# fizzy74/passport-zk-circuits

Hardware: AMD Instinct MI355X
Metric: registerIdentityBuilder witnesses/sec, batch=4096, 1 & 8 MI355X; % HBM roofline (higher is better)
Workload: dtype bn254_fr (u32 limbs)

## Files before the change

passport-zk-circuits_amd/csrc/kernels_rsa.hip:

```cpp
#include <hip/hip_runtime.h>
#include <stdio.h>
#include <stdlib.h>

#define PZK_TEMPLATE_KERNELS_ONLY
#include "regemit.hpp"
#include "rsa_coop.hpp"
#include "kernels.hpp"

namespace pzk {

#define HIP_TRY(x) do { hipError_t e_ = (x); if (e_ != hipSuccess) return e_; } while (0)

template <int K, int G>
static hipError_t launch_rsa_core2(const DevLayout& L, const uint8_t* inputs, uint64_t* rsa_core, int32_t* status,
                                   uint32_t batch, hipStream_t st) {
  constexpr int WPB = 64 / G;
  const size_t lds = sizeof(uint64_t) * rsa2_lds_words<K>() * WPB;
  HIP_TRY(hipFuncSetAttribute((const void*)k_rsa_core2<K, G>, hipFuncAttributeMaxDynamicSharedMemorySize, (int)lds));
  hipLaunchKernelGGL((k_rsa_core2<K, G>), dim3((batch + WPB - 1) / WPB), dim3(64), lds, st, L, inputs, rsa_core, status,
                     batch);
  return hipGetLastError();
}

template <int K, int NL>
static hipError_t launch_rsa_lane(const DevLayout& L, const uint8_t* inputs, uint64_t* rsa_core, uint64_t* colsum,
                                  int32_t* status, uint32_t batch, hipStream_t st) {
  const size_t lds = sizeof(uint64_t) * rsa_lds_words<K>() * NL;
  HIP_TRY(hipFuncSetAttribute((const void*)k_rsa_core<K, NL>, hipFuncAttributeMaxDynamicSharedMemorySize, (int)lds));
  hipLaunchKernelGGL((k_rsa_core<K, NL>), dim3((batch + NL - 1) / NL), dim3(NL), lds, st, L, inputs, rsa_core, colsum,
                     status, batch);
  return hipGetLastError();
}

static bool rsa_core_lane() {
  static const int v = [] {
    const char* e = getenv("PZK_RSA_CORE");
    return e && e[0] == 'l' ? 1 : 0;
  }();
  return v;
}

hipError_t launch_rsa_core(const DevLayout& L, const uint8_t* inputs, uint64_t* rsa_core, uint64_t* colsum,
                           int32_t* status, uint32_t batch, hipStream_t st) {
  const bool lane = rsa_core_lane() && colsum;
  if (L.reg.K == 48) {
    HIP_TRY((launch_rsa_core2<48, 16>(L, inputs, rsa_core, status, batch, st)));
    hipLaunchKernelGGL(k_rsa_inv<48>, dim3((batch + RI_WAVES - 1) / RI_WAVES), dim3(64 * RI_WAVES), 0, st, L, inputs,
                       rsa_core, batch);
  } else if (L.reg.K == 32) {
    HIP_TRY((lane ? launch_rsa_lane<32, 64>(L, inputs, rsa_core, colsum, status, batch, st)
                  : launch_rsa_core2<32, 8>(L, inputs, rsa_core, status, batch, st)));
    hipLaunchKernelGGL(k_rsa_inv<32>, dim3((batch + RI_WAVES - 1) / RI_WAVES), dim3(64 * RI_WAVES), 0, st, L, inputs,
                       rsa_core, batch);
  } else {
    HIP_TRY((lane ? launch_rsa_lane<64, 32>(L, inputs, rsa_core, colsum, status, batch, st)
                  : launch_rsa_core2<64, 16>(L, inputs, rsa_core, status, batch, st)));
    hipLaunchKernelGGL(k_rsa_inv<64>, dim3((batch + RI_WAVES - 1) / RI_WAVES), dim3(64 * RI_WAVES), 0, st, L, inputs,
                       rsa_core, batch);
  }
  return hipGetLastError();
}

hipError_t launch_emit_mm(const DevLayout& L, const Work* work, uint32_t n_work, const Bufs& B, uint32_t batch,
                          hipStream_t st) {
#ifdef PZK_MM_PROF
  {
    static int n = 0;
    if (++n > 1) {
      unsigned long long h[MM_SECTIONS + 2];
      if (hipDeviceSynchronize() == hipSuccess && hipMemcpyFromSymbol(h, HIP_SYMBOL(g_mm_prof), sizeof h) == hipSuccess) {
        fprintf(stderr, "mm_prof launches=%d", n - 1);
        for (int i = 0; i <= (int)MM_SECTIONS; i++) fprintf(stderr, " %llu", h[i]);
        fprintf(stderr, "\n");
      }
    }
  }
#endif
  if (n_work == 0) return hipSuccess;
  const bool m = L.keep.bits != nullptr;
  static const bool wide = !getenv("PZK_MM_THREADS") || atoi(getenv("PZK_MM_THREADS")) != 256;
  const bool w512 = wide && !m && L.reg.K == 32;
  dim3 g(n_work, batch), blk(w512 ? 512 : EMIT_THREADS);
  auto kern = w512 ? k_emit_mm<32, MAP_O0, 512>
            : L.reg.K == 32 ? (m ? k_emit_mm<32, MAP_DIRECT> : k_emit_mm<32, MAP_O0>)
            : L.reg.K == 48 ? (m ? k_emit_mm<48, MAP_DIRECT> : k_emit_mm<48, MAP_O0>)
                            : (m ? k_emit_mm<64, MAP_DIRECT> : k_emit_mm<64, MAP_O0>);
  hipLaunchKernelGGL(kern, g, blk, 0, st, L, work, B);
  return hipGetLastError();
}

}
```

passport-zk-circuits_amd/csrc/regcore.hpp:

```cpp
#pragma once
#include "fr.hpp"
#include "layout.hpp"
#include "poseidon.hpp"
#include "sha.hpp"
#include "core_util.hpp"
#include "pss.hpp"

namespace pzk {

__device__ __forceinline__ fr wave_bits_fr(const uint8_t* row, int base, int L, int dir, bool& bad) {
  const int lane = threadIdx.x & 63;
  fr v = fr_zero();
  for (int q = 0; 64 * q < L; q++) {
    const int k = 64 * q + lane;
    uint32_t b = 0;
    if (k < L) b = in_bit(row, dir > 0 ? base + k : base + L - 1 - k, bad);
    const uint64_t m = __ballot(b);
    v.v[2 * q] = (uint32_t)m;
    v.v[2 * q + 1] = (uint32_t)(m >> 32);
  }
  return v;
}

#ifndef PZK_TEMPLATE_KERNELS_ONLY
// ... 106 lines not shown
    n[i] = in_u64(e);
  }
  int nb = K;
  while (nb > 1 && n[nb - 1] == 0) nb--;
  const int s = __builtin_clzll(n[nb - 1] | 1ull);
  for (int i = nb - 1; i > 0; i--) vn[i] = (n[i] << s) | (s ? n[i - 1] >> (64 - s) : 0ull);
  vn[0] = n[0] << s;
  const uint64_t vtop = vn[nb - 1], vsec = nb > 1 ? vn[nb - 2] : 0ull;
  uint64_t vinv_r;
  const uint64_t vinv = vtop ? divlu(~vtop, ~0ull, vtop, &vinv_r) : 0ull;
  constexpr int MMW = MM_CORE_WORDS(K);
  const int NM = L.reg.n_modmul;
  for (int k = 0; k < NM; k++) {
    uint64_t* mc = core + (size_t)k * MMW;
    for (int i = 0; i < K; i++) {
      uint64_t xi;
      const int sx = L.reg.mm_x[k], sy = L.reg.mm_y[k];
      if (sx < 0) {
        const uint8_t* e = row + 32ull * (L.reg.in_sig + i);
        bad |= !in_is_u64(e);
        xi = in_u64(e);
      } else {
        xi = core[(size_t)sx * MMW + 3 * K + 1 + i];
      }
      uint64_t yi = sy == sx ? xi : core[(size_t)sy * MMW + 3 * K + 1 + i];
      x[i] = xi; y[i] = yi;
      mc[i] = xi; mc[K + i] = yi;
    }
    {
      uint64_t c0 = 0, c1 = 0;
      for (int i = 0; i < 2 * K; i++) {
        U192 acc;
        int lo = i < K ? 0 : i - K + 1, hi = i < K ? i : K - 1;
        for (int j = lo; j <= hi; j++) acc.mac(x[j], y[i - j]);
        if (i < 2 * K - 1) { CS(i, 0) = acc.a0; CS(i, 1) = acc.a1; CS(i, 2) = acc.a2; }
        uint64_t t0 = acc.a0 + c0; uint64_t cc = t0 < c0;
        uint64_t t1 = acc.a1 + c1; uint64_t cc1 = t1 < c1; uint64_t t1b = t1 + cc; cc1 += t1b < t1;
        u[i] = t0; c0 = t1b; c1 = acc.a2 + cc1;
      }
    }
    u[2 * K] = s ? u[2 * K - 1] >> (64 - s) : 0ull;
    if (s) {
      for (int i = 2 * K - 1; i > 0; i--) u[i] = (u[i] << s) | (u[i - 1] >> (64 - s));
      u[0] = u[0] << s;
    }
    for (int j = 0; j <= K; j++) q[j] = 0;
    for (int j = 2 * K - nb; j >= 0 && vtop; j--) {
      uint64_t ujn = u[j + nb], ujn1 = u[j + nb - 1];
      uint64_t qhat, rhat;
      bool rhat_ovf = false;
      if (ujn >= vtop) {
        qhat = ~0ull;
        rhat = ujn1 + vtop;
        rhat_ovf = rhat < ujn1;
      } else {
        qhat = div_preinv(ujn, ujn1, vtop, vinv, &rhat);
      }
      if (nb > 1) {
        for (int it = 0; it < 2 && !rhat_ovf; it++) {
          uint64_t plo = qhat * vsec, phi = __umul64hi(qhat, vsec);
          uint64_t u2 = u[j + nb - 2];
          if (phi > rhat || (phi == rhat && plo > u2)) {
            qhat--;
            uint64_t r2 = rhat + vtop;
            rhat_ovf = r2 < rhat;
            rhat = r2;
          } else {
            break;
          }
        }
      }
      uint64_t borrow = 0, carry = 0;
      for (int i = 0; i < nb; i++) {
        uint64_t plo = qhat * vn[i], phi = __umul64hi(qhat, vn[i]);
        plo += carry; phi += plo < carry; carry = phi;
        uint64_t t = u[i + j];
        uint64_t d = t - plo; uint64_t b1 = t < plo;
        uint64_t d2 = d - borrow; uint64_t b2 = d < borrow;
        u[i + j] = d2; borrow = b1 + b2;
      }
      uint64_t t = u[j + nb];
      uint64_t d = t - carry; uint64_t b1 = t < carry;
      uint64_t d2 = d - borrow; uint64_t b2 = d < borrow;
      u[j + nb] = d2;
      if (b1 + b2) {
        qhat--;
        uint64_t cy = 0;
        for (int i = 0; i < nb; i++) {
          uint64_t a = u[i + j], vb = vn[i];
          uint64_t sm = a + vb; uint64_t ca = sm < a; uint64_t sm2 = sm + cy; uint64_t cb = sm2 < sm;
          u[i + j] = sm2; cy = ca + cb;
        }
        u[j + nb] += cy;
      }
      q[j] = qhat;
    }
    uint64_t* qo = mc + 2 * K;
    uint64_t* ro = mc + 3 * K + 1;
    for (int i = 0; i <= K; i++) qo[i] = q[i];
    for (int i = 0; i < K; i++) {
      uint64_t r = 0;
      if (i < nb) r = s ? (u[i] >> s) | (u[i + 1] << (64 - s)) : u[i];
      ro[i] = r;
    }
    uint64_t* cr = mc + 8 * K + 1;
    {
      uint64_t clo = 0, chi = 0;
      for (int i = 0; i < 2 * K - 1; i++) {
        U192 a, b;
        a.a0 = CS(i, 0); a.a1 = CS(i, 1); a.a2 = CS(i, 2);
        int lo2 = i < K ? 0 : i - K + 1, hi2 = i < K + 1 ? i : K;
        for (int j = lo2; j <= hi2 && j <= K; j++) if (i - j < K) b.mac(q[j], n[i - j]);
        uint64_t s0, s1, s2, s3, br;
        s0 = a.a0 - b.a0; br = a.a0 < b.a0;
        uint64_t t1 = a.a1 - b.a1; uint64_t br1 = a.a1 < b.a1; s1 = t1 - br; br1 += t1 < br; br = br1;
        uint64_t t2 = a.a2 - b.a2; uint64_t br2 = a.a2 < b.a2; s2 = t2 - br; br2 += t2 < br; br = br2;
        s3 = 0 - br;
        uint64_t rr = i < K ? ro[i] : 0ull;
        uint64_t u0 = s0 - rr; uint64_t bb = s0 < rr; s0 = u0;
        uint64_t u1 = s1 - bb; bb = s1 < bb; s1 = u1;
        uint64_t u2 = s2 - bb; bb = s2 < bb; s2 = u2; s3 -= bb;
        uint64_t csx = (int64_t)chi < 0 ? ~0ull : 0ull;
        uint64_t v0 = s0 + clo; uint64_t cc = v0 < s0;
        uint64_t v1 = s1 + chi; uint64_t cc1 = v1 < s1; uint64_t v1b = v1 + cc; cc1 += v1b < v1;
        uint64_t v2 = s2 + csx; uint64_t cc2 = v2 < s2; uint64_t v2b = v2 + cc1; cc2 += v2b < v2;
        uint64_t v3 = s3 + csx + cc2;
        if (i < 2 * K - 2) {
          badz |= v0 != 0;
          clo = v1b; chi = v2b;
          badz |= !((v3 == 0 && (int64_t)v2b >= 0) || (v3 == ~0ull && (int64_t)v2b < 0));
          cr[2 * i] = clo; cr[2 * i + 1] = chi;
        } else {
          badz |= (v0 | v1b | v2b | v3) != 0;
        }
      }
    }
  }
  if (bad || !vtop) set_status(status, ST_INPUT_RANGE);
  if (badz) set_status(status, ST_BIGISZERO);
}

template <int K, int NL>
__global__ void __launch_bounds__(NL) k_rsa_core(DevLayout L, const uint8_t* inputs, uint64_t* rsa_core, uint64_t* colsum,
                                                 int32_t* status, uint32_t batch) {
  core_priority();
  extern __shared__ uint64_t lds_rsa[];
  uint32_t w = blockIdx.x * NL + threadIdx.x;
  if (w >= batch) return;
  rsa_lane<K, NL>(L, inputs + 32ull * (uint64_t)w * L.n_inputs, rsa_core + (size_t)w * L.rsa_core_words, colsum + w,
                  batch, status ? status + w : nullptr, lds_rsa, threadIdx.x);
}

#ifndef PZK_RI_WAVES
#define PZK_RI_WAVES 8
#endif
constexpr int RI_WAVES = PZK_RI_WAVES;
template <int J, int N, class F>
__device__ __forceinline__ void static_for(F&& f) {
  if constexpr (J < N) {
    f(std::integral_constant<int, J>{});
    static_for<J + 1, N>(f);
  }
}
template <int K>
__global__ void __launch_bounds__(64 * RI_WAVES) k_rsa_inv(DevLayout L, const uint8_t* inputs, uint64_t* rsa_core,
                                                           uint32_t batch) {
  core_priority();
  constexpr int PER_MAX = (20 * K + 63) / 64 < 12 ? (20 * K + 63) / 64 : 12;
  __shared__ fr s_tot[RI_WAVES];
  __shared__ fr s_out[RI_WAVES][64];
  const int wv = (int)(threadIdx.x >> 6), lane = (int)(threadIdx.x & 63);
  const uint32_t w0 = blockIdx.x * RI_WAVES + (uint32_t)wv;
  const bool live = w0 < batch;
  const uint32_t w = live ? w0 : batch - 1;
  const int NE = L.reg.n_modmul * K, PER = (NE + 63) / 64, in_pk = (int)L.reg.in_pk;
  constexpr int MMW = MM_CORE_WORDS(K);
  const uint8_t* row = inputs + 32ull * (uint64_t)w * L.n_inputs;
  uint64_t* core = rsa_core + (size_t)w * L.rsa_core_words;
  const int e0 = lane * PER, e1 = !live ? e0 : e0 + PER < NE ? e0 + PER : NE;
  auto diff = [=](int e) -> fr {
    const int k = e / K, i = e - k * K;
    const uint64_t a = core[(size_t)k * MMW + 3 * K + 1 + i], b = in_u64(row + 32ull * (in_pk + i));
    fr d = a >= b ? fr_u64(a - b) : fr_sub(fr_zero(), fr_u64(b - a));
    return fr_to_mont(d);
  };
  auto slot = [=](int e) -> uint8_t* {
    const int k = e / K, i = e - k * K;
    return reinterpret_cast<uint8_t*>(core + (size_t)k * MMW + 4 * K + 1 + 4 * i);
  };
  const bool in_reg = PER <= PER_MAX;
  fr pr[PER_MAX];
  fr acc = fr_mont_one();
  if (in_reg) {
    static_for<0, PER_MAX>([&](auto J) __attribute__((always_inline)) {
      const int e = e0 + J();
      if (e < e1) {
        const fr d = diff(e);
        pr[J()] = acc;
        if (!fr_is_zero(d)) acc = fr_mul_fast(acc, d);
      }
    });
  } else {
    for (int e = e0; e < e1; e++) {
      const fr d = diff(e);
      store_fr(slot(e), acc);
      if (!fr_is_zero(d)) acc = fr_mul_fast(acc, d);
    }
  }
  fr incl = acc, sincl = acc;
  for (int d = 1; d < 64; d <<= 1) {
    fr a = fr_shfl_up(incl, d), b = fr_shfl_down(sincl, d);
    if (lane >= d) incl = fr_mul_fast(incl, a);
    if (lane + d < 64) sincl = fr_mul_fast(sincl, b);
  }
  fr pre = fr_shfl_up(incl, 1), suf = fr_shfl_down(sincl, 1);
  if (lane == 0) pre = fr_mont_one();
  if (lane == 63) suf = fr_mont_one();
  if (lane == 63) s_tot[wv] = incl;
  __syncthreads();
  if (wv == 0) {
    const fr t = lane < RI_WAVES ? s_tot[lane] : fr_mont_one();
    fr t_others, t_all;
    fr_group_others<RI_WAVES>(t, t_others, t_all);
    const fr t_inv = fr_mul_fast(fr_inv<true>(t_all), t_others);
    if (lane < RI_WAVES) s_tot[lane] = t_inv;
  }
  __syncthreads();
  fr inv = fr_mul_fast(fr_mul_fast(s_tot[wv], pre), suf);
  if (!in_reg) {
    if (!live) return;
    for (int e = e1 - 1; e >= e0; e--) {
      const fr d = diff(e);
      fr r = fr_zero();
      if (!fr_is_zero(d)) { r = fr_mul_fast(inv, load_fr(slot(e))); inv = fr_mul_fast(inv, d); }
      store_fr(slot(e), fr_from_mont(r));
    }
    return;
  }
  static_for<0, PER_MAX>([&](auto J) __attribute__((always_inline)) {
    constexpr int j = PER_MAX - 1 - J();
    const int e = e0 + j;
    if (e < e1) {
      const fr d = diff(e);
      fr r = fr_zero();
      if (!fr_is_zero(d)) { r = fr_mul_fast(inv, pr[j]); inv = fr_mul_fast(inv, d); }
      pr[j] = fr_from_mont(r);
    }
  });
  for (int t = 0; t < (NE + 63) / 64; t++) {
    static_for<0, PER_MAX>([&](auto J) __attribute__((always_inline)) {
      const int e = e0 + J();
      if (e < e1 && (e >> 6) == t) s_out[wv][e & 63] = pr[J()];
    });
    __syncthreads();
    const int e = 64 * t + lane;
    if (live && e < NE) store_fr(slot(e), s_out[wv][lane]);
    __syncthreads();
  }
}

constexpr uint64_t RSA_EM4 = 217300885422736416ull, RSA_EM5 = 938447882527703397ull;
constexpr uint64_t RSA_EM6 = 0xFFFFFFFF00303130ull;

#ifndef PZK_TEMPLATE_KERNELS_ONLY
__global__ void __launch_bounds__(64) k_rsa_check(DevLayout L, const uint8_t* inputs, const uint32_t* sha_core,
                                                  const uint64_t* rsa_core, int32_t* status, uint32_t batch) {
  const uint32_t w = blockIdx.x * blockDim.x + threadIdx.x;
  if (w >= batch || !status) return;
  const int K = L.reg.K;
  const uint8_t* row = inputs + 32ull * (uint64_t)w * L.n_inputs;
  const uint64_t* core = rsa_core + (size_t)w * L.rsa_core_words;
  const uint64_t* em = core + (size_t)(L.reg.n_modmul - 1) * MM_CORE_WORDS(K) + 3 * K + 1;
  const ShaJob& J = L.sha[L.reg.j_sa];
  const uint32_t* H = sha_core + (size_t)w * L.sha_core_words + J.hout;
  bool hash_bad = false;
  for (int i = 0; i < 4; i++) {
    const int wd = 3 - i;
    hash_bad |= (((uint64_t)H[2 * wd] << 32) | H[2 * wd + 1]) != em[i];
  }
  bool pad_bad = em[6] != RSA_EM6;
  for (int i = 7; i < K - 1; i++) pad_bad |= em[i] != ~0ull;
  bool gt_bad = false;
  for (int m = 0; m < L.reg.n_modmul; m++) {
    const uint64_t* r = core + (size_t)m * MM_CORE_WORDS(K) + 3 * K + 1;
    int cmp = 0;
    for (int i = K - 1; i >= 0 && cmp == 0; i--) {
      uint64_t n = in_u64(row + 32ull * (L.reg.in_pk + i));
      cmp = n > r[i] ? 1 : n < r[i] ? -1 : 0;
    }
    gt_bad |= cmp != 1;
  }
  if (L.reg.pss_s8) {
    pss_check(pss_view(L, rsa_core, sha_core, w), status + w);
  } else if (J.algo == 1) {
    const uint64_t em2 = em[2];
    if ((uint32_t)em2 != H[0]) lane_status(status + w, ST_RSA_HASH);
    if ((em2 >> 32) != 83887124ull || em[3] != 650212878678426138ull || em[4] != 18446744069417738544ull)
      lane_status(status + w, ST_RSA_PREFIX);
    bool pb = em[K - 1] != 562949953421311ull;
    for (int i = 5; i < K - 1; i++) pb |= em[i] != ~0ull;
    if (pb) lane_status(status + w, ST_RSA_PAD);
  } else {
    if (hash_bad) lane_status(status + w, ST_RSA_HASH);
    if (em[4] != RSA_EM4 || em[5] != RSA_EM5) lane_status(status + w, ST_RSA_PREFIX);
    if (pad_bad) lane_status(status + w, ST_RSA_PAD);
  }
  if (gt_bad) lane_status(status + w, ST_BIGMOD_GT);
}
#endif

struct ExtPt { fr X, Y, Z, T; };

template <class PM = FrMulInline>
__device__ __forceinline__ ExtPt bjj_dbl(const ExtPt& P, const fr& A) {
  fr a = PM::sqr(P.X), b = PM::sqr(P.Y), c = PM::sqr(P.Z);
  c = fr_add(c, c);
  fr d = PM::mul(A, a);
  fr xy = fr_add(P.X, P.Y);
  fr e = fr_sub(fr_sub(PM::sqr(xy), a), b);
  fr g = fr_add(d, b), f = fr_sub(g, c), h = fr_sub(d, b);
  return ExtPt{PM::mul(e, f), PM::mul(g, h), PM::mul(f, g), PM::mul(e, h)};
}
template <class PM = FrMulInline>
__device__ __forceinline__ ExtPt bjj_add_affine(const ExtPt& P, const fr& x2, const fr& y2, const fr& t2d, const fr& A) {
  fr a = PM::mul(P.X, x2), b = PM::mul(P.Y, y2), c = PM::mul(P.T, t2d), d = P.Z;
  fr e = fr_sub(fr_sub(PM::mul(fr_add(P.X, P.Y), fr_add(x2, y2)), a), b);
  fr f = fr_sub(d, c), g = fr_add(d, c), h = fr_sub(b, PM::mul(A, a));
  return ExtPt{PM::mul(e, f), PM::mul(g, h), PM::mul(f, g), PM::mul(e, h)};
}

constexpr uint32_t BJJ_B8X[8] = {0xbb957051u, 0x2893f3f6u, 0x0534e0b6u, 0x2ab8d801u,
                                 0x9d6277c1u, 0x4eacb2e0u, 0xd63e739bu, 0x0bb77a6au};
constexpr uint32_t BJJ_B8Y[8] = {0x872d7d8bu, 0x4b3c257au, 0xb9e13377u, 0xfce0051fu,
                                 0xd16bf9edu, 0x25572e1cu, 0xf7a0b249u, 0x25797203u};
constexpr uint32_t BJJ_INV_B8X[8] = {0x7bc45854u, 0x42cd5135u, 0x5936d873u, 0x5dc5f319u,
                                     0x40d1c783u, 0x40e2c828u, 0xcaabb2bdu, 0x0b1a7dddu};
constexpr uint64_t BJJ_A = 168700, BJJ_D = 168696;

constexpr uint32_t BJJ_M_A[8] = {0xfff261e0u, 0x95accf61u, 0x9df7d378u, 0x24780d65u,
                                 0x7e906ae8u, 0xe0ac11b0u, 0x16d3def3u, 0x0f35db22u};
constexpr uint32_t BJJ_M_D[8] = {0xaff261f5u, 0x2735f484u, 0x9a2e0f63u, 0x70ba1b57u,
                                 0x1e2caa8cu, 0xff41c9a9u, 0x8fe6025fu, 0x07704a8eu};
constexpr uint32_t BJJ_M_B8X[8] = {0x1a89fa86u, 0x0a8fc7bcu, 0xe9e48627u, 0xa7d9d786u,
                                   0x65bea369u, 0xee6158b4u, 0x2f874519u, 0x14a0ff6du};
constexpr uint32_t BJJ_M_B8Y[8] = {0x0d0201aau, 0xb83342d2u, 0xcdcfeac7u, 0x2ffef2f7u,
                                   0x25a6e625u, 0xbfa79a94u, 0xc3a44b70u, 0x0dfb859du};
constexpr uint32_t BJJ_M_B8TD[8] = {0x0f1b2ee0u, 0x10c75c99u, 0xc23309edu, 0x83d5e20cu,
                                    0xe93991cfu, 0x3fc6be6bu, 0xb5195112u, 0x03a44577u};

struct BjjConsts {
  fr A, D, B8x, B8y, B8t_d;
  __device__ __forceinline__ void init() {
    A = fr_to_mont(fr_u64(BJJ_A)); D = fr_to_mont(fr_u64(BJJ_D));
    B8x = fr_to_mont(fr_const(BJJ_B8X)); B8y = fr_to_mont(fr_const(BJJ_B8Y));
    B8t_d = fr_mul(fr_mul(D, B8x), B8y);
  }
  __device__ __forceinline__ void init_literal() {
    A = fr_const(BJJ_M_A); D = fr_const(BJJ_M_D);
    B8x = fr_const(BJJ_M_B8X); B8y = fr_const(BJJ_M_B8Y); B8t_d = fr_const(BJJ_M_B8TD);
  }
};

template <class PM = FrMulInline>
__device__ __forceinline__ ExtPt bjj_add(const ExtPt& P, const ExtPt& Q, const BjjConsts& C) {
  fr a = PM::mul(P.X, Q.X), b = PM::mul(P.Y, Q.Y), c = PM::mul(PM::mul(P.T, C.D), Q.T), d = PM::mul(P.Z, Q.Z);
  fr e = fr_sub(fr_sub(PM::mul(fr_add(P.X, P.Y), fr_add(Q.X, Q.Y)), a), b);
  fr f = fr_sub(d, c), g = fr_add(d, c), h = fr_sub(b, PM::mul(C.A, a));
  return ExtPt{PM::mul(e, f), PM::mul(g, h), PM::mul(f, g), PM::mul(e, h)};
}

#ifndef PZK_TEMPLATE_KERNELS_ONLY
__global__ void __launch_bounds__(256) k_bjj_table(fr* table) {
  const int idx = blockIdx.x * blockDim.x + threadIdx.x;
  if (idx >= BJJ_TABLE_WINDOWS * 256) return;
  const int wi = idx >> 8, v = idx & 255;
  BjjConsts C;
  C.init();
  fr* out = table + 3 * (size_t)idx;
  if (v == 0) { out[0] = fr_zero(); out[1] = fr_zero(); out[2] = fr_zero(); return; }
  ExtPt base{C.B8x, C.B8y, fr_mont_one(), fr_mul(C.B8x, C.B8y)};
  for (int k = 0; k < 8 * wi; k++) base = bjj_dbl(base, C.A);
  ExtPt acc = base;
  for (int bit = 30 - __clz(v); bit >= 0; bit--) {
    acc = bjj_dbl(acc, C.A);
    if ((v >> bit) & 1) acc = bjj_add(acc, base, C);
  }
  fr zi = fr_inv(acc.Z);
  fr x = fr_mul(acc.X, zi), y = fr_mul(acc.Y, zi);
  out[0] = x; out[1] = y; out[2] = fr_mul(fr_mul(C.D, x), y);
}
#endif


template <class PM = FrMulInline>
__device__ __forceinline__ void bjj_seg_start(const fr& sk, int i0, const fr* table, const BjjConsts& C, bool& have,
                                              ExtPt& A) {
  have = false;
  A = ExtPt{fr_zero(), fr_zero(), fr_zero(), fr_zero()};
  for (int wi = 0; 8 * wi < i0; wi++) {
    uint32_t v = 0;
    for (int b = 0; b < 8 && 8 * wi + b < i0; b++) v |= fr_bit(sk, 254 - i0 + 8 * wi + b) << b;
    if (!v) continue;
    const fr* e = table + 3 * (size_t)(wi * 256 + v);
    if (!have) { A = ExtPt{e[0], e[1], fr_mont_one(), PM::mul(e[0], e[1])}; have = true; }
    else A = bjj_add_affine<PM>(A, e[0], e[1], e[2], C.A);
  }
}
template <int SEGS, int SEG_LEN, class PM = FrMulInline>
__device__ __forceinline__ void bjj_seg_start_paired(const fr& sk, int seg, const fr* table, const BjjConsts& C,
                                                     bool& have, ExtPt& A) {
// ... 384 lines not shown
```

passport-zk-circuits_amd/csrc/runtime.cpp:

```cpp
#include <dlfcn.h>
#include <hip/hip_runtime.h>
#include <stdio.h>
#include <string.h>

#include <algorithm>
#include <atomic>
#include <map>
#include <mutex>
#include <string>
#include <vector>

#include "../../include/pzkwit.h"
#include "builder.hpp"
#include "kernels.hpp"
#include "bufs.hpp"
#include "ec_common.hpp"
#include "poseidon.hpp"
#include "query_layout.hpp"
#include "host_api.hpp"

using namespace pzk;

static thread_local std::string g_err;
static int fail(int code, const std::string& msg) { g_err = msg; return code; }
// ... 875 lines not shown
      s_emit = I->s_post;
    }
    { PhaseScope ps(T, slot, PH_PREP, st); HIPCHK(launch_qry_prep(L, d_inputs, vs, d_status, st)); }
    { PhaseScope ps(T, slot, PH_BJJ_CORE, st);
      HIPCHK(launch_bjj_core(L, vs, I->d_bjj_table, S.d_bjj_core, S.d_bjj_scratch, st)); }
    HIPCHK(hipEventRecord(I->ev_bjj, st));
    HIPCHK(hipStreamWaitEvent(s_sha, I->ev_bjj, 0));
    if ((rc = emit(E_BJJ, s_sha))) return rc;
    { PhaseScope ps(T, slot, PH_POS_CORE, st); if ((rc = pos_levels(0, 4))) return rc; }
    { PhaseScope ps(T, slot, PH_SMT, st); HIPCHK(launch_smt_prep(L, d_inputs, vs, S.d_smt_core, d_status, st));
      HIPCHK(launch_smt_order(S.d_smt_core, L.smt_core_fr, S.d_smt_order, B, st)); }
    { PhaseScope ps(T, slot, PH_POS_CORE, st); if ((rc = pos_levels(4, 6, S.d_smt_order))) return rc; }
    static const bool emit1 = getenv("PZK_QRY_EMIT1") != nullptr;
    hipStream_t s_pe = emit1 ? s_sha : s_emit;
    static const bool split = [] { const char* e = getenv("PZK_QRY_SPLIT"); return e ? atoi(e) != 0 : true; }();
    if (split) {
      HIPCHK(hipEventRecord(I->ev_pos, st));
      HIPCHK(hipStreamWaitEvent(s_pe, I->ev_pos, 0));
      if ((rc = emit(E_POS, s_pe, 0, lay.pos_chain_group))) return rc;
      HIPCHK(hipStreamWaitEvent(s_sha, I->ev_pos, 0));
      if ((rc = emit(E_QRY, s_sha))) return rc;
      if ((rc = emit(E_BITS, s_sha))) return rc;
      if ((rc = emit(E_GEN, s_sha, 0, lay.gen_chain_work))) return rc;
    }
    { PhaseScope ps(T, slot, PH_SMT, st);
      HIPCHK(launch_smt_chain(L, K, I->d_level_task, d_inputs, vs, S.d_pos_core, S.d_smt_core, S.d_smt_order, d_status,
                              st)); }
    HIPCHK(hipEventRecord(I->ev_chain, st));
    HIPCHK(hipStreamWaitEvent(s_pe, I->ev_chain, 0));
    if ((rc = emit(E_POS, s_pe, split ? lay.pos_chain_group : 0))) return rc;
    HIPCHK(hipStreamWaitEvent(s_sha, I->ev_chain, 0));
    if ((rc = emit(E_GEN, s_sha, split ? lay.gen_chain_work : 0))) return rc;
    if (!split) {
      if ((rc = emit(E_QRY, s_sha))) return rc;
      if ((rc = emit(E_BITS, s_sha))) return rc;
    }
  } else if (lay.is_light) {
    HIPCHK(hipEventRecord(I->ev_load, st));
    HIPCHK(hipStreamWaitEvent(s_rsa, I->ev_load, 0));
    { PhaseScope ps(T, slot, PH_SHA_CORE, s_rsa);
      HIPCHK(launch_sha_core(L, d_inputs, S.d_derived, 0, L.n_sha, S.d_sha_core, d_status, B, s_rsa)); }
    HIPCHK(hipEventRecord(I->ev_sha, s_rsa));
    { PhaseScope ps(T, slot, PH_PREP, s_rsa); HIPCHK(launch_light_prep(L, d_inputs, S.d_sha_core, vs, d_status, s_rsa)); }
    HIPCHK(hipEventRecord(I->ev_rsa, s_rsa));
    { PhaseScope ps(T, slot, PH_BJJ_CORE, st);
      HIPCHK(launch_bjj_core(L, vs, I->d_bjj_table, S.d_bjj_core, S.d_bjj_scratch, st)); }
    HIPCHK(hipEventRecord(I->ev_bjj, st));
    { PhaseScope ps(T, slot, PH_POS_CORE, st); if ((rc = pos_levels(0, 1))) return rc; }
    HIPCHK(hipStreamWaitEvent(st, I->ev_rsa, 0));
    { PhaseScope ps(T, slot, PH_POS_CORE, st); if ((rc = pos_levels(1, 1 << 20))) return rc; }
    HIPCHK(hipEventRecord(I->ev_pos, st));
    HIPCHK(hipStreamWaitEvent(s_sha, I->ev_sha, 0));
    if ((rc = emit(E_SHA, s_sha))) return rc;
    if ((rc = emit(E_SHA1, s_sha))) return rc;
    if ((rc = emit(E_SHA5, s_sha))) return rc;
    HIPCHK(hipStreamWaitEvent(s_emit, I->ev_bjj, 0));
    if ((rc = emit(E_BJJ, s_emit))) return rc;
    HIPCHK(hipStreamWaitEvent(s_emit, I->ev_pos, 0));
    if ((rc = emit(E_POS, s_emit))) return rc;
    if ((rc = emit(E_BITS, s_emit))) return rc;
    if ((rc = emit(E_GEN, s_emit))) return rc;
  } else if (!lay.is_register) {
    static const char* ov_env = getenv("PZK_OVERLAP");
    const bool overlap = ov_env ? atoi(ov_env) != 0 : L.n_sha == 0;
    if (!overlap) s_emit = st;
    { PhaseScope ps(T, slot, PH_SHA_CORE, st);
      HIPCHK(launch_sha_core(L, d_inputs, S.d_derived, 0, L.n_sha, S.d_sha_core, d_status, B, st)); }
    { PhaseScope ps(T, slot, PH_POS_CORE, st); if ((rc = pos_levels(0, 1 << 20))) return rc; }
    if (s_emit != st) {
      HIPCHK(hipEventRecord(I->ev_pos, st));
      HIPCHK(hipStreamWaitEvent(s_emit, I->ev_pos, 0));
    }
    for (int e = 0; e < E_COUNT; e++)
      if ((rc = emit(e, s_emit))) return rc;
    s_rsa = s_sha = s_own = st;
  } else {
    HIPCHK(hipEventRecord(I->ev_load, st));
    HIPCHK(hipStreamWaitEvent(s_rsa, I->ev_load, 0));
    const bool pss = lay.reg.pss_s8 != 0;
    const uint32_t n_sha_main = pss ? (uint32_t)lay.reg.j_mgf : (uint32_t)lay.sha.size();
    if (!lay.is_ecdsa) {
      PhaseScope ps(T, slot, PH_RSA_CORE, s_rsa);
      HIPCHK(launch_rsa_core(L, d_inputs, S.d_rsa_core, S.d_rsa_colsum, d_status, B, s_rsa));
    }
    { PhaseScope ps(T, slot, PH_SHA_CORE, st);
      HIPCHK(launch_sha_core(L, d_inputs, S.d_derived, 0, n_sha_main, S.d_sha_core, d_status, B, st)); }
    HIPCHK(hipEventRecord(I->ev_sha, st));
    if (pss) {
      HIPCHK(hipStreamWaitEvent(s_rsa, I->ev_sha, 0));
      PhaseScope ps(T, slot, PH_PSS, s_rsa);
      HIPCHK(launch_pss(L, 0, S.d_rsa_core, S.d_sha_core, S.d_derived, B, s_rsa));
      HIPCHK(launch_sha_core(L, d_inputs, S.d_derived, (uint32_t)lay.reg.j_mgf, (uint32_t)lay.reg.n_mgf,
                             S.d_sha_core, d_status, B, s_rsa));
      HIPCHK(launch_pss(L, 1, S.d_rsa_core, S.d_sha_core, S.d_derived, B, s_rsa));
      HIPCHK(launch_sha_core(L, d_inputs, S.d_derived, (uint32_t)lay.reg.j_hd, 1, S.d_sha_core, d_status, B,
                             s_rsa));
    }
    if (lay.is_ecdsa) {
      HIPCHK(hipStreamWaitEvent(s_rsa, I->ev_sha, 0));
      { PhaseScope ps(T, slot, PH_EC_CORE, s_rsa);
        HIPCHK(launch_ec_core(L, d_inputs, S.d_sha_core, S.d_ec_core, S.d_ec_jac, S.d_ec_inv, d_status, B, s_rsa)); }
    }
    HIPCHK(hipEventRecord(I->ev_rsa, s_rsa));
    if (lay.is_ecdsa) {
      { PhaseScope ps(T, slot, PH_EC_TABLE, s_rsa);
        for (int t = 0; t < 3; t++)
          HIPCHK(launch_ec_table(L, t, I->d_ec_ops[t], (uint32_t)lay.ec_ops[t].size(), S.d_ec_core, S.d_ec_tab,
                                 d_status, B, s_rsa)); }
      HIPCHK(hipEventRecord(I->ev_tab, s_rsa));
    }
    HIPCHK(hipStreamWaitEvent(s_sha, I->ev_sha, 0));
    if ((rc = emit(E_SHA, s_sha))) return rc;
    if ((rc = emit(E_SHA1, s_sha))) return rc;
    if ((rc = emit(E_SHA5, s_sha))) return rc;
    static const char* se_env = getenv("PZK_SIGEMIT");
    const bool sig_on_rsa = se_env ? strcmp(se_env, "emit") != 0 : !lay.is_ecdsa;
    hipStream_t s_sig = I->s_mm && !serial ? I->s_mm : sig_on_rsa ? s_rsa : s_emit;
    HIPCHK(hipStreamWaitEvent(s_sig, I->ev_rsa, 0));
    if ((rc = emit(E_MM, s_sig))) return rc;
    if ((rc = emit(E_SHAD, s_sig))) return rc;
    if ((rc = emit(E_SHA5D, s_sig))) return rc;
    if (lay.is_ecdsa) {
      if ((rc = emit(E_ECR, s_sig))) return rc;
      HIPCHK(hipStreamWaitEvent(s_sig, I->ev_tab, 0));
      if ((rc = emit(E_ECT, s_sig, 0, ect_split))) return rc;
    }
    { PhaseScope ps(T, slot, PH_PREP, st); HIPCHK(launch_prep(L, d_inputs, S.d_sha_core, vs, d_status, st)); }
    { PhaseScope ps(T, slot, PH_POS_CORE, st); if ((rc = pos_levels(0, 2))) return rc; }
    { PhaseScope ps(T, slot, PH_SMT, st); HIPCHK(launch_smt_prep(L, d_inputs, vs, S.d_smt_core, d_status, st));
      HIPCHK(launch_smt_order(S.d_smt_core, L.smt_core_fr, S.d_smt_order, B, st)); }
    { PhaseScope ps(T, slot, PH_POS_CORE, st); if ((rc = pos_levels(2, 3, S.d_smt_order))) return rc; }
    static const char* tail_env = getenv("PZK_TAIL");
    static const int tail_mode = !tail_env ? 2 : !strcmp(tail_env, "emit") ? 1 : !strcmp(tail_env, "sha") ? 0
                                 : !strcmp(tail_env, "rsa") ? 3 : !strcmp(tail_env, "own") ? 4 : 2;
    static const char* smt_env = getenv("PZK_SMT");
    static const int smt_mode = !smt_env ? 1 : !strcmp(smt_env, "main") ? 0 : !strcmp(smt_env, "tail") ? 2 : 1;
    static const int smt_chains = getenv("PZK_SMT_CHAINS") ? atoi(getenv("PZK_SMT_CHAINS")) : 2;
    const hipStream_t chain_streams[3] = {I->s_tail, I->s_chain2, I->s_chain3};
    const int n_chain = smt_chains < 1 ? 1 : smt_chains >= 3 && I->s_chain3 ? 3 : smt_chains >= 2 ? 2 : 1;
    hipStream_t s_smt = (serial || tail_mode == 4 || smt_mode == 0) ? st : chain_streams[I->chain_rr++ % n_chain];
    if (s_smt != st) {
      HIPCHK(hipEventRecord(I->ev_smt, st));
      HIPCHK(hipStreamWaitEvent(s_smt, I->ev_smt, 0));
    }
    { PhaseScope ps(T, slot, PH_SMT, s_smt);
      HIPCHK(launch_smt_chain(L, K, I->d_level_task, d_inputs, vs, S.d_pos_core, S.d_smt_core, S.d_smt_order, d_status,
                              s_smt)); }
    HIPCHK(hipEventRecord(I->ev_chain, s_smt));
    { PhaseScope ps(T, slot, PH_BJJ_CORE, st);
      HIPCHK(launch_bjj_core(L, vs, I->d_bjj_table, S.d_bjj_core, S.d_bjj_scratch, st)); }
    HIPCHK(hipEventRecord(I->ev_bjj, st));
    { PhaseScope ps(T, slot, PH_POS_CORE, st); if ((rc = pos_levels(3, 1 << 20))) return rc; }
    HIPCHK(hipEventRecord(I->ev_pos, st));
    hipStream_t s_tail = tail_mode == 1 ? s_emit : tail_mode == 3 ? s_rsa : tail_mode == 4 ? s_own : s_sha,
                s_pos = tail_mode == 0 ? s_sha : s_emit, s_bjj = tail_mode == 4 ? s_own : s_sha;
    if (s_smt != st && smt_mode == 2) s_tail = s_smt;
    HIPCHK(hipStreamWaitEvent(s_bjj, I->ev_bjj, 0));
    if ((rc = emit(E_BJJ, s_bjj))) return rc;
    const bool post = I->s_post && !serial && s_smt != st;
    const uint32_t pos_split = post ? lay.pos_chain_group : ~0u, gen_split = post ? lay.gen_chain_work : ~0u;
    HIPCHK(hipStreamWaitEvent(s_pos, I->ev_pos, 0));
    if (!post && s_smt != st && s_pos != s_smt) HIPCHK(hipStreamWaitEvent(s_pos, I->ev_chain, 0));
    if ((rc = emit(E_POS, s_pos, 0, pos_split))) return rc;
    HIPCHK(hipStreamWaitEvent(s_tail, I->ev_pos, 0));
    HIPCHK(hipStreamWaitEvent(s_tail, I->ev_rsa, 0));
    if (!post && s_smt != st && s_tail != s_smt) HIPCHK(hipStreamWaitEvent(s_tail, I->ev_chain, 0));
    if ((rc = emit(E_GEN, s_tail, 0, gen_split))) return rc;
    if (post) {
      HIPCHK(hipStreamWaitEvent(I->s_post, I->ev_pos, 0));
      HIPCHK(hipStreamWaitEvent(I->s_post, I->ev_chain, 0));
      if ((rc = emit(E_POS, I->s_post, pos_split))) return rc;
      if ((rc = emit(E_GEN, I->s_post, gen_split))) return rc;
    }
    if ((rc = emit(E_FLOW, s_tail))) return rc;
    if (!lay.is_ecdsa) {
      PhaseScope ps(T, slot, PH_PREP, s_tail);
      HIPCHK(launch_rsa_check(L, d_inputs, S.d_sha_core, S.d_rsa_core, d_status, B, s_tail));
    }
    if ((rc = emit(E_BITS, s_tail))) return rc;
    if ((rc = emit(E_GENR, s_tail))) return rc;
    if (lay.is_ecdsa && ect_split < lay.work[E_ECT].size()) {
      HIPCHK(hipStreamWaitEvent(s_sha, I->ev_tab, 0));
      if ((rc = emit(E_ECT, s_sha, ect_split))) return rc;
    }
  }
  auto or_st = [&](hipStream_t s) { return serial || !s ? st : s; };
  hipStream_t streams[pzk_instance::NSTREAMS] = {st, s_rsa, s_sha, s_emit, s_own, or_st(I->s_chain2),
                                                 or_st(I->s_chain3), or_st(I->s_post), or_st(I->s_mm), st};
  for (int i = 0; i < pzk_instance::NSTREAMS; i++) HIPCHK(hipEventRecord(I->ev_done[set][i], streams[i]));
  if (user) {
    for (hipEvent_t e : I->ev_done[set]) HIPCHK(hipStreamWaitEvent(user, e, 0));
  }
  if (exec && (exec->flags & PZK_EXEC_SYNC)) {
    if (user) HIPCHK(hipStreamSynchronize(user));
    else if ((rc = sync_all(I))) return rc;
  }
  return 0;
}

static constexpr size_t MAP_CHUNK = 1024, MAP_CHUNK_MIN = 64;
static int batch_mapped(pzk_instance* I, const uint8_t* d_inputs, size_t batch, uint8_t* d_wtns, size_t stride,
                        int32_t* d_status, const pzk_exec* exec, const uint8_t* d_packed = nullptr) {
  const size_t o0_stride = 32ull * I->lay.wit_size;
  size_t chunk = std::min(batch, MAP_CHUNK);
  if (chunk > I->o0_cap) {
    int rc = sync_all(I);
    if (rc) return rc;
    for (auto& p : I->d_o0) { if (p) (void)hipFree(p); p = nullptr; }
    I->o0_cap = 0;
    for (;;) {
      bool ok = true;
      for (auto& p : I->d_o0) ok = ok && hipMalloc(&p, o0_stride * chunk) == hipSuccess;
      if (ok) break;
      for (auto& p : I->d_o0) { if (p) (void)hipFree(p); p = nullptr; }
      (void)hipGetLastError();
      if (chunk <= MAP_CHUNK_MIN) return fail(PZK_E_NOMEM, "device O0 staging allocation failed");
      chunk /= 2;
    }
    I->o0_cap = chunk;
  }
  chunk = std::min(chunk, I->o0_cap);
  hipStream_t user = (exec && exec->stream) ? (hipStream_t)exec->stream : nullptr;
  if (user) {
    HIPCHK(hipEventRecord(I->ev_entry, user));
    HIPCHK(hipStreamWaitEvent(I->stream, I->ev_entry, 0));
  }
  pzk_exec ex{I->device, exec ? (exec->flags & PZK_EXEC_TIMING) : 0, nullptr};
  for (size_t lo = 0; lo < batch; lo += chunk) {
    const size_t n = std::min(chunk, batch - lo);
    const int set = (int)(I->calls % I->nsets), slot = (int)((lo / chunk) & 1);
    HIPCHK(hipStreamWaitEvent(I->stream, I->ev_gather[slot], 0));
    int rc = batch_locked(I, d_packed ? nullptr : d_inputs + 32ull * I->lay.n_inputs * lo, n, I->d_o0[slot], o0_stride,
                          d_status ? d_status + lo : nullptr, &ex, I->stream,
                          d_packed ? d_packed + I->packed.row_bytes * lo : nullptr);
    if (rc) return rc;
    for (int i = 0; i < pzk_instance::NSTREAMS; i++) HIPCHK(hipStreamWaitEvent(I->stream, I->ev_done[set][i], 0));
    HIPCHK(launch_wtns_gather(I->d_o0[slot], o0_stride, I->d_map, I->out_size, d_wtns + stride * lo, stride, (uint32_t)n,
                              I->stream));
    HIPCHK(hipEventRecord(I->ev_done[set][0], I->stream));
    HIPCHK(hipEventRecord(I->ev_gather[slot], I->stream));
  }
  if (user)
    for (auto& set : I->ev_done)
      for (hipEvent_t e : set) HIPCHK(hipStreamWaitEvent(user, e, 0));
  if (exec && (exec->flags & PZK_EXEC_SYNC)) {
    if (user) HIPCHK(hipStreamSynchronize(user));
    else return sync_all(I);
  }
  return 0;
}

static int pzk_witness_batch_impl(pzk_instance* I, const uint8_t* d_inputs, size_t batch, uint8_t* d_wtns, size_t stride,
                      int32_t* d_status, const pzk_exec* exec, bool packed = false) {
  if (!I || !d_inputs || !d_wtns) return fail(PZK_E_ARG, "null argument");
  if (packed && (uintptr_t)d_inputs % 16) return fail(PZK_E_ARG, "packed rows must be 16-byte aligned");
  if (batch == 0) return 0;
  if (batch > 65535) return fail(PZK_E_ARG, "batch > 65535: split it");
  if (stride < 32ull * I->out_size || stride % 16) return fail(PZK_E_ARG, "bad witness stride");
  int rc = check_exec_device(I, exec);
  if (rc) return rc;
  std::lock_guard<std::mutex> lock(I->mu);
  DeviceGuard dg(I->device);
  if (dg.err != hipSuccess) return fail(PZK_E_HIP, std::string("hipSetDevice: ") + hipGetErrorString(dg.err));
  if (packed) {
    if (I->d_map) return batch_mapped(I, nullptr, batch, d_wtns, stride, d_status, exec, d_inputs);
    return batch_locked(I, nullptr, batch, d_wtns, stride, d_status, exec, nullptr, d_inputs);
  }
  if (I->d_map) return batch_mapped(I, d_inputs, batch, d_wtns, stride, d_status, exec);
  return batch_locked(I, d_inputs, batch, d_wtns, stride, d_status, exec);
}

static int pzk_unpack_inputs_impl(pzk_instance* I, const uint8_t* d_packed, size_t batch, uint8_t* d_rows,
                                  const pzk_exec* exec) {
  if (!I || !d_packed || !d_rows) return fail(PZK_E_ARG, "null argument");
  if (batch == 0) return 0;
  if (batch > 65535) return fail(PZK_E_ARG, "batch > 65535: split it");
  if ((uintptr_t)d_packed % 16 || (uintptr_t)d_rows % 16) return fail(PZK_E_ARG, "packed rows and rows must be 16-byte aligned");
  int rc = check_exec_device(I, exec);
  if (rc) return rc;
  std::lock_guard<std::mutex> lock(I->mu);
  DeviceGuard dg(I->device);
  if (dg.err != hipSuccess) return fail(PZK_E_HIP, std::string("hipSetDevice: ") + hipGetErrorString(dg.err));
  if ((rc = ensure_in_rows(I, nullptr, 0))) return rc;
  hipStream_t st = (exec && exec->stream) ? (hipStream_t)exec->stream : I->stream;
  HIPCHK(launch_unpack_inputs(I->d_packed_groups, (uint32_t)I->packed.groups.size(), I->lay.n_inputs, I->packed.row_bytes,
                              d_packed, d_rows, (uint32_t)batch, st));
  if (exec && (exec->flags & PZK_EXEC_SYNC)) HIPCHK(hipStreamSynchronize(st));
  return 0;
}

static int pzk_instance_input_packed_impl(const pzk_instance* I, uint32_t i, uint32_t* kind, uint64_t* off, uint64_t* len) {
  if (!I || i >= I->packed.groups.size()) return fail(PZK_E_ARG, "input index out of range");
  const PackedGroup& g = I->packed.groups[i];
  if (kind) *kind = g.kind;
  if (off) *off = g.byte_off;
  if (len) *len = packed_group_bytes(g.kind, g.elem_len);
  return 0;
}

static int pzk_instance_sync_impl(pzk_instance* I) {
  if (!I) return fail(PZK_E_ARG, "null argument");
  std::lock_guard<std::mutex> lock(I->mu);
  DeviceGuard dg(I->device);
  if (dg.err != hipSuccess) return fail(PZK_E_HIP, std::string("hipSetDevice: ") + hipGetErrorString(dg.err));
  return sync_all(I);
}

static int pzk_witness_batch_host_impl(pzk_instance* I, const uint8_t* h_inputs, size_t batch, uint8_t* h_wtns,
                           int32_t* h_status, const pzk_exec* exec, bool packed = false) {
  if (!I || !h_inputs || !h_wtns) return fail(PZK_E_ARG, "null argument");
  if (batch == 0) return 0;
  if (batch > 65535) return fail(PZK_E_ARG, "batch > 65535: split it");
  int rc = check_exec_device(I, exec);
  if (rc) return rc;
  std::lock_guard<std::mutex> lock(I->mu);
  DeviceGuard dg(I->device);
// ... 244 lines not shown
```

Measured before the change: 82990.

## Rework RSA batch-inverse kernel with strided elements and checkpointed prefixes; retune tail streams

The RSA Montgomery batch-inversion kernel now specialises PER at compile time through a launcher. Each lane takes elements strided by 64 instead of a contiguous block, so stores to the core buffer coalesce directly and the LDS staging loop with its repeated __syncthreads is gone. Only every second or third prefix product is kept in registers and the missing ones are recomputed on the way back, which trades extra multiplies and reloads for lower register pressure. It also drops waves per block from 8 to 4, replaces the group reduction with a serial product, and in the default RSA path moves the BJJ emit onto the emit stream after POS.

```diff
diff --git a/passport-zk-circuits_amd/csrc/kernels_rsa.hip b/passport-zk-circuits_amd/csrc/kernels_rsa.hip
--- a/passport-zk-circuits_amd/csrc/kernels_rsa.hip
+++ b/passport-zk-circuits_amd/csrc/kernels_rsa.hip
@@ -40,23 +40,30 @@
   return v;
 }
 
+template <int K>
+static void launch_rsa_inv(const DevLayout& L, const uint8_t* inputs, uint64_t* rsa_core, uint32_t batch, hipStream_t st) {
+  constexpr int P17 = ri_per(K, 17), P20 = ri_per(K, 20);
+  const int per = ri_per(K, L.reg.n_modmul);
+  const dim3 g((batch + RI_WAVES - 1) / RI_WAVES), blk(64 * RI_WAVES);
+  if (K <= 48 && per <= P17) hipLaunchKernelGGL((k_rsa_inv<K, K <= 48 ? P17 : 0>), g, blk, 0, st, L, inputs, rsa_core, batch);
+  else if (K <= 48 && per <= P20) hipLaunchKernelGGL((k_rsa_inv<K, K <= 48 ? P20 : 0>), g, blk, 0, st, L, inputs, rsa_core, batch);
+  else hipLaunchKernelGGL((k_rsa_inv<K, 0>), g, blk, 0, st, L, inputs, rsa_core, batch);
+}
+
 hipError_t launch_rsa_core(const DevLayout& L, const uint8_t* inputs, uint64_t* rsa_core, uint64_t* colsum,
                            int32_t* status, uint32_t batch, hipStream_t st) {
   const bool lane = rsa_core_lane() && colsum;
   if (L.reg.K == 48) {
     HIP_TRY((launch_rsa_core2<48, 16>(L, inputs, rsa_core, status, batch, st)));
-    hipLaunchKernelGGL(k_rsa_inv<48>, dim3((batch + RI_WAVES - 1) / RI_WAVES), dim3(64 * RI_WAVES), 0, st, L, inputs,
-                       rsa_core, batch);
+    launch_rsa_inv<48>(L, inputs, rsa_core, batch, st);
   } else if (L.reg.K == 32) {
     HIP_TRY((lane ? launch_rsa_lane<32, 64>(L, inputs, rsa_core, colsum, status, batch, st)
                   : launch_rsa_core2<32, 8>(L, inputs, rsa_core, status, batch, st)));
-    hipLaunchKernelGGL(k_rsa_inv<32>, dim3((batch + RI_WAVES - 1) / RI_WAVES), dim3(64 * RI_WAVES), 0, st, L, inputs,
-                       rsa_core, batch);
+    launch_rsa_inv<32>(L, inputs, rsa_core, batch, st);
   } else {
     HIP_TRY((lane ? launch_rsa_lane<64, 32>(L, inputs, rsa_core, colsum, status, batch, st)
                   : launch_rsa_core2<64, 16>(L, inputs, rsa_core, status, batch, st)));
-    hipLaunchKernelGGL(k_rsa_inv<64>, dim3((batch + RI_WAVES - 1) / RI_WAVES), dim3(64 * RI_WAVES), 0, st, L, inputs,
-                       rsa_core, batch);
+    launch_rsa_inv<64>(L, inputs, rsa_core, batch, st);
   }
   return hipGetLastError();
 }
diff --git a/passport-zk-circuits_amd/csrc/regcore.hpp b/passport-zk-circuits_amd/csrc/regcore.hpp
--- a/passport-zk-circuits_amd/csrc/regcore.hpp
+++ b/passport-zk-circuits_amd/csrc/regcore.hpp
@@ -282,9 +282,10 @@
 }
 
 #ifndef PZK_RI_WAVES
-#define PZK_RI_WAVES 8
+#define PZK_RI_WAVES 4
 #endif
 constexpr int RI_WAVES = PZK_RI_WAVES;
+constexpr int ri_ck(int K) { return K <= 32 ? 2 : 3; }
 template <int J, int N, class F>
 __device__ __forceinline__ void static_for(F&& f) {
   if constexpr (J < N) {
@@ -292,100 +293,110 @@
     static_for<J + 1, N>(f);
   }
 }
-template <int K>
+constexpr int ri_per(int K, int n_modmul) { return (n_modmul * K + 63) / 64; }
+template <int K, int PER>
 __global__ void __launch_bounds__(64 * RI_WAVES) k_rsa_inv(DevLayout L, const uint8_t* inputs, uint64_t* rsa_core,
                                                            uint32_t batch) {
   core_priority();
-  constexpr int PER_MAX = (20 * K + 63) / 64 < 12 ? (20 * K + 63) / 64 : 12;
   __shared__ fr s_tot[RI_WAVES];
-  __shared__ fr s_out[RI_WAVES][64];
   const int wv = (int)(threadIdx.x >> 6), lane = (int)(threadIdx.x & 63);
   const uint32_t w0 = blockIdx.x * RI_WAVES + (uint32_t)wv;
   const bool live = w0 < batch;
   const uint32_t w = live ? w0 : batch - 1;
-  const int NE = L.reg.n_modmul * K, PER = (NE + 63) / 64, in_pk = (int)L.reg.in_pk;
+  const int NE = live ? L.reg.n_modmul * K : 0, in_pk = (int)L.reg.in_pk;
   constexpr int MMW = MM_CORE_WORDS(K);
   const uint8_t* row = inputs + 32ull * (uint64_t)w * L.n_inputs;
   uint64_t* core = rsa_core + (size_t)w * L.rsa_core_words;
-  const int e0 = lane * PER, e1 = !live ? e0 : e0 + PER < NE ? e0 + PER : NE;
-  auto diff = [=](int e) -> fr {
+  auto diff = [=](int e) __attribute__((always_inline)) -> fr {
     const int k = e / K, i = e - k * K;
     const uint64_t a = core[(size_t)k * MMW + 3 * K + 1 + i], b = in_u64(row + 32ull * (in_pk + i));
     fr d = a >= b ? fr_u64(a - b) : fr_sub(fr_zero(), fr_u64(b - a));
     return fr_to_mont(d);
   };
-  auto slot = [=](int e) -> uint8_t* {
+  auto slot = [=](int e) __attribute__((always_inline)) -> uint8_t* {
     const int k = e / K, i = e - k * K;
     return reinterpret_cast<uint8_t*>(core + (size_t)k * MMW + 4 * K + 1 + 4 * i);
   };
-  const bool in_reg = PER <= PER_MAX;
-  fr pr[PER_MAX];
+  constexpr int RI_CK = ri_ck(K);
+  constexpr int NCK = PER > 0 ? (PER + RI_CK - 1) / RI_CK : 1;
+  fr ck[NCK];
   fr acc = fr_mont_one();
-  if (in_reg) {
-    static_for<0, PER_MAX>([&](auto J) __attribute__((always_inline)) {
-      const int e = e0 + J();
-      if (e < e1) {
+  if constexpr (PER > 0) {
+    static_for<0, PER>([&](auto J) __attribute__((always_inline)) {
+      constexpr int j = J();
+      __builtin_amdgcn_sched_barrier(0);
+      const int e = 64 * j + lane;
+      if (e < NE) {
         const fr d = diff(e);
-        pr[J()] = acc;
+        if constexpr (j % RI_CK == 0) ck[j / RI_CK] = acc;
         if (!fr_is_zero(d)) acc = fr_mul_fast(acc, d);
       }
     });
   } else {
-    for (int e = e0; e < e1; e++) {
+    for (int e = lane; e < NE; e += 64) {
       const fr d = diff(e);
       store_fr(slot(e), acc);
       if (!fr_is_zero(d)) acc = fr_mul_fast(acc, d);
     }
   }
-  fr incl = acc, sincl = acc;
+  fr pre = acc;
   for (int d = 1; d < 64; d <<= 1) {
-    fr a = fr_shfl_up(incl, d), b = fr_shfl_down(sincl, d);
-    if (lane >= d) incl = fr_mul_fast(incl, a);
-    if (lane + d < 64) sincl = fr_mul_fast(sincl, b);
-  }
-  fr pre = fr_shfl_up(incl, 1), suf = fr_shfl_down(sincl, 1);
+    const fr a = fr_shfl_up(pre, d);
+    if (lane >= d) pre = fr_mul_fast(pre, a);
+  }
+  if (lane == 63) s_tot[wv] = pre;
+  pre = fr_shfl_up(pre, 1);
   if (lane == 0) pre = fr_mont_one();
+  fr suf = acc;
+  for (int d = 1; d < 64; d <<= 1) {
+    const fr b = fr_shfl_down(suf, d);
+    if (lane + d < 64) suf = fr_mul_fast(suf, b);
+  }
+  suf = fr_shfl_down(suf, 1);
   if (lane == 63) suf = fr_mont_one();
-  if (lane == 63) s_tot[wv] = incl;
+  fr inv = fr_mul_fast(pre, suf);
   __syncthreads();
   if (wv == 0) {
-    const fr t = lane < RI_WAVES ? s_tot[lane] : fr_mont_one();
-    fr t_others, t_all;
-    fr_group_others<RI_WAVES>(t, t_others, t_all);
+    fr t_all = fr_mont_one(), t_others = fr_mont_one();
+    for (int k = 0; k < RI_WAVES; k++) {
+      const fr t = s_tot[k];
+      t_all = fr_mul_fast(t_all, t);
+      if (k != lane) t_others = fr_mul_fast(t_others, t);
+    }
     const fr t_inv = fr_mul_fast(fr_inv<true>(t_all), t_others);
+    __builtin_amdgcn_wave_barrier();
     if (lane < RI_WAVES) s_tot[lane] = t_inv;
   }
   __syncthreads();
-  fr inv = fr_mul_fast(fr_mul_fast(s_tot[wv], pre), suf);
-  if (!in_reg) {
-    if (!live) return;
-    for (int e = e1 - 1; e >= e0; e--) {
+  inv = fr_mul_fast(s_tot[wv], inv);
+  if constexpr (PER > 0) {
+    static_for<0, PER>([&](auto J) __attribute__((always_inline)) {
+      constexpr int j = PER - 1 - J(), j0 = j - j % RI_CK;
+      __builtin_amdgcn_sched_barrier(0);
+      const int e = 64 * j + lane;
+      if (e < NE) {
+        const fr d = diff(e);
+        fr r = fr_zero();
+        if (!fr_is_zero(d)) {
+          fr p = ck[j0 / RI_CK];
+          static_for<j0, j>([&](auto I) __attribute__((always_inline)) {
+            const fr di = diff(64 * I() + lane);
+            if (!fr_is_zero(di)) p = fr_mul_fast(p, di);
+          });
+          r = fr_mul_fast(inv, p);
+          inv = fr_mul_fast(inv, d);
+        }
+        store_fr(slot(e), fr_from_mont(r));
+      }
+    });
+  } else {
+    for (int j = (NE > lane ? (NE - lane + 63) / 64 : 0) - 1; j >= 0; j--) {
+      const int e = 64 * j + lane;
       const fr d = diff(e);
       fr r = fr_zero();
       if (!fr_is_zero(d)) { r = fr_mul_fast(inv, load_fr(slot(e))); inv = fr_mul_fast(inv, d); }
       store_fr(slot(e), fr_from_mont(r));
     }
-    return;
-  }
-  static_for<0, PER_MAX>([&](auto J) __attribute__((always_inline)) {
-    constexpr int j = PER_MAX - 1 - J();
-    const int e = e0 + j;
-    if (e < e1) {
-      const fr d = diff(e);
-      fr r = fr_zero();
-      if (!fr_is_zero(d)) { r = fr_mul_fast(inv, pr[j]); inv = fr_mul_fast(inv, d); }
-      pr[j] = fr_from_mont(r);
-    }
-  });
-  for (int t = 0; t < (NE + 63) / 64; t++) {
-    static_for<0, PER_MAX>([&](auto J) __attribute__((always_inline)) {
-      const int e = e0 + J();
-      if (e < e1 && (e >> 6) == t) s_out[wv][e & 63] = pr[J()];
-    });
-    __syncthreads();
-    const int e = 64 * t + lane;
-    if (live && e < NE) store_fr(slot(e), s_out[wv][lane]);
-    __syncthreads();
   }
 }
 
diff --git a/passport-zk-circuits_amd/csrc/runtime.cpp b/passport-zk-circuits_amd/csrc/runtime.cpp
--- a/passport-zk-circuits_amd/csrc/runtime.cpp
+++ b/passport-zk-circuits_amd/csrc/runtime.cpp
@@ -1051,16 +1051,24 @@
     HIPCHK(hipEventRecord(I->ev_bjj, st));
     { PhaseScope ps(T, slot, PH_POS_CORE, st); if ((rc = pos_levels(3, 1 << 20))) return rc; }
     HIPCHK(hipEventRecord(I->ev_pos, st));
-    hipStream_t s_tail = tail_mode == 1 ? s_emit : tail_mode == 3 ? s_rsa : tail_mode == 4 ? s_own : s_sha,
-                s_pos = tail_mode == 0 ? s_sha : s_emit, s_bjj = tail_mode == 4 ? s_own : s_sha;
+    const bool tail_emit = !tail_env && !serial && !lay.is_ecdsa && !I->on_pool && !I->chain_set_shared &&
+                           !(I->s_sha2 && I->sha2_on);
+    hipStream_t s_tail = tail_mode == 1 || tail_emit ? s_emit : tail_mode == 3 ? s_rsa : tail_mode == 4 ? s_own : s_sha,
+                s_pos = tail_mode == 0 ? s_sha : s_emit, s_bjj = tail_emit ? s_emit : tail_mode == 4 ? s_own : s_sha;
     if (s_smt != st && smt_mode == 2) s_tail = s_smt;
-    HIPCHK(hipStreamWaitEvent(s_bjj, I->ev_bjj, 0));
-    if ((rc = emit(E_BJJ, s_bjj))) return rc;
+    if (!tail_emit) {
+      HIPCHK(hipStreamWaitEvent(s_bjj, I->ev_bjj, 0));
+      if ((rc = emit(E_BJJ, s_bjj))) return rc;
+    }
     const bool post = I->s_post && !serial && s_smt != st;
     const uint32_t pos_split = post ? lay.pos_chain_group : ~0u, gen_split = post ? lay.gen_chain_work : ~0u;
     HIPCHK(hipStreamWaitEvent(s_pos, I->ev_pos, 0));
     if (!post && s_smt != st && s_pos != s_smt) HIPCHK(hipStreamWaitEvent(s_pos, I->ev_chain, 0));
     if ((rc = emit(E_POS, s_pos, 0, pos_split))) return rc;
+    if (tail_emit) {
+      HIPCHK(hipStreamWaitEvent(s_bjj, I->ev_bjj, 0));
+      if ((rc = emit(E_BJJ, s_bjj))) return rc;
+    }
     HIPCHK(hipStreamWaitEvent(s_tail, I->ev_pos, 0));
     HIPCHK(hipStreamWaitEvent(s_tail, I->ev_rsa, 0));
     if (!post && s_smt != st && s_tail != s_smt) HIPCHK(hipStreamWaitEvent(s_tail, I->ev_chain, 0));
```

Result: no change. 82970, median of 4 (-0.0%).
